# DanielLin94144/E2E-ASR-Pytorch

Hardware: NVIDIA B200
Metric: beam-8+LM joint CTC/attn decode utts/sec (higher is better)
Workload: dtype f32

## Files before the change

### e2e-asr-pytorch_b200/_lib.py

```python
import ctypes
import os

from . import build as _build

c_int, c_float, c_void_p = ctypes.c_int, ctypes.c_float, ctypes.c_void_p

CTC_LOGZERO = -100000000.0
DEC_LOG_ZERO = -10000000.0
STATUS_PREFIX_TOO_LONG = 1
STATUS_TOKEN_NOT_CAND = 2
PREFIX_FULL = 1
PREFIX_SKIP_DEAD_ROWS = 2
PREFIX_FAST_MATH = 4
PREFIX_LIBM_MATH = 8
PREFIX_ROW_COPIES = 16
PREFIX_POLY_MATH = 32
PREFIX_POLY_ESTRIN = 64
BEAM_USE_CTC = 1
BEAM_USE_LM = 2

SIGNATURES = {
    "e2e_last_error": (ctypes.c_char_p, []),
    "e2e_abi_version": (c_int, []),
    "e2e_padded_vocab": (c_int, [c_int]),
# ... 37 lines not shown
    "e2e_lstm_cell": (c_int, [c_void_p, ctypes.c_longlong, c_void_p, c_void_p, c_void_p, c_void_p, c_void_p, c_int, c_int,
                              c_void_p, c_void_p, c_void_p, ctypes.c_longlong, c_int, c_int, c_void_p]),
    "e2e_lstm_split_rows_f16x2": (c_int, [c_void_p, ctypes.c_longlong, c_void_p, c_int, c_int, c_void_p, ctypes.c_longlong, c_int, c_int,
                                          c_float, c_void_p]),
    "e2e_lstm_split_rows_multi_f16x2": (c_int, [c_int, c_void_p, c_void_p, c_void_p, c_void_p, c_void_p, c_void_p, c_void_p, c_void_p,
                                                c_int, c_float, c_void_p]),
    "e2e_lstm_cell_f16x2": (c_int, [c_void_p, ctypes.c_longlong, c_float, c_void_p, c_void_p, c_void_p, c_void_p, c_void_p, c_int, c_int,
                                    c_void_p, c_void_p, c_void_p, ctypes.c_longlong, c_int, c_int, c_float, c_void_p]),
    "e2e_gru_cell": (c_int, [c_void_p, ctypes.c_longlong, c_void_p, c_void_p, c_void_p, c_void_p, c_void_p, c_int, c_int,
                             c_void_p, c_void_p, ctypes.c_longlong, c_int, c_int, c_void_p]),
    "e2e_gru_cell_f16x2": (c_int, [c_void_p, ctypes.c_longlong, c_float, c_void_p, c_void_p, c_void_p, c_void_p, c_void_p, c_int, c_int,
                                   c_void_p, c_void_p, ctypes.c_longlong, c_int, c_int, c_float, c_void_p]),
    "e2e_conv3x3_unfold_split": (c_int, [c_void_p, c_void_p, c_int, c_int, c_int, c_int, ctypes.c_longlong, c_int, c_void_p, c_void_p]),
    "e2e_conv_bias_relu_mask": (c_int, [c_void_p, c_void_p, c_void_p, c_int, c_int, c_int, c_int, ctypes.c_longlong,
                                        ctypes.c_longlong, c_void_p]),
    "e2e_lstm_sequence": (c_int, [c_void_p, ctypes.c_longlong, c_void_p, ctypes.c_longlong, c_void_p, c_void_p, c_void_p, c_void_p,
                                  c_int, c_int, c_int, c_int,
                                  c_void_p, c_void_p, c_int, c_int, c_void_p, c_void_p, c_int, c_int, c_void_p]),
    "e2e_gru_sequence": (c_int, [c_void_p, ctypes.c_longlong, c_void_p, ctypes.c_longlong, c_void_p, c_void_p, c_void_p, c_void_p,
                                 c_int, c_int, c_int, c_int,
                                 c_void_p, c_void_p, c_int, c_int, c_void_p, c_void_p, c_int, c_int, c_void_p]),
    "e2e_conv1_direct": (c_int, [c_void_p, ctypes.c_longlong, c_void_p, c_void_p, c_void_p, c_int, c_int, c_int, c_int, c_int,
                                 c_void_p, c_void_p]),
    "e2e_conv_bias_relu_mask_pool": (c_int, [c_void_p, c_void_p, c_void_p, c_int, c_int, c_int, c_int, c_void_p, c_void_p]),
    "e2e_conv1_direct_amax": (c_int, [c_void_p, ctypes.c_longlong, c_void_p, c_void_p, c_void_p, c_int, c_int, c_int, c_int, c_int,
                                      c_void_p, c_void_p, c_void_p]),
    "e2e_conv3x3_unfold_split_f16x2": (c_int, [c_void_p, c_void_p, c_int, c_int, c_int, c_int, ctypes.c_longlong, c_int, c_void_p,
                                               c_void_p, c_void_p]),
    "e2e_conv_bias_relu_mask_scaled": (c_int, [c_void_p, c_void_p, c_void_p, c_int, c_int, c_int, c_int, ctypes.c_longlong,
                                               ctypes.c_longlong, c_void_p, c_float, c_void_p, c_void_p]),
# ... 53 lines not shown
```

### e2e-asr-pytorch_b200/build.py

```python
import os
import shutil
import subprocess

_HERE = os.path.dirname(os.path.abspath(__file__))
CSRC = os.path.join(_HERE, "csrc")
LIB_DIR = os.path.join(_HERE, "lib")
LIB_PATH = os.path.join(LIB_DIR, "libe2e_asr_b200.so")
SOURCES = ["abi.cu", "ctc_posterior.cu", "prefix_score.cu", "prefix_lazy.cu", "beam_step.cu", "attention_full.cu", "lstm_step.cu", "conv_split.cu", "lstm_seq.cu"]
HEADERS = [os.path.join(CSRC, "common.cuh"), os.path.join(CSRC, "softplus_lut.inc"), os.path.join(CSRC, "softplus_poly.inc"), os.path.join(_HERE, "..", "include", "e2e_asr_b200.h")]
NVCC_FLAGS = ["-gencode", "arch=compute_100a,code=sm_100a", "-O3", "-lineinfo", "-std=c++17",
              "--expt-extended-lambda", "-Xcompiler", "-fPIC", "-shared"]


def _nvcc():
    for cand in (os.environ.get("NVCC"), shutil.which("nvcc"), "/usr/local/cuda/bin/nvcc"):
        if cand and os.path.exists(cand):
            return cand
    return None


def stale():
    if not os.path.exists(LIB_PATH):
        return True
    built = os.path.getmtime(LIB_PATH)
    deps = [os.path.join(CSRC, s) for s in SOURCES] + HEADERS
    return any(os.path.getmtime(d) > built for d in deps)


def build(force=False, verbose=False):
    if not force and not stale():
        return LIB_PATH
    nvcc = _nvcc()
    if nvcc is None:
        raise RuntimeError("nvcc not found: cannot build libe2e_asr_b200.so")
    import tempfile
    from concurrent.futures import ThreadPoolExecutor
    os.makedirs(LIB_DIR, exist_ok=True)
    compile_flags = [f for f in NVCC_FLAGS if f != "-shared"] + (["-Xptxas", "-v"] if verbose else [])
    with tempfile.TemporaryDirectory(prefix="e2e_build_") as tmp:
        def compile_one(src):
            obj = os.path.join(tmp, src.replace(".cu", ".o"))
            proc = subprocess.run([nvcc] + compile_flags + ["-c", "-o", obj, src], cwd=CSRC, capture_output=True, text=True)
            return src, obj, proc
        with ThreadPoolExecutor(max_workers=min(len(SOURCES), os.cpu_count() or 1)) as pool:
            done = list(pool.map(compile_one, SOURCES))
        failed = [(src, proc) for src, _, proc in done if proc.returncode != 0]
        if failed:
            raise RuntimeError("nvcc failed:\n" + "\n".join(src + ":\n" + proc.stdout + proc.stderr for src, proc in failed))
        if verbose:
            for src, _, proc in done:
                print(proc.stderr)
        out_tmp = LIB_PATH + ".tmp%d" % os.getpid()
        link = subprocess.run([nvcc] + NVCC_FLAGS + ["-o", out_tmp] + [obj for _, obj, _ in done], cwd=CSRC, capture_output=True, text=True)
        if link.returncode != 0:
            raise RuntimeError("nvcc link failed:\n" + link.stdout + link.stderr)
        os.replace(out_tmp, LIB_PATH)
    return LIB_PATH


if __name__ == "__main__":
    print(build(force=True, verbose=True))
```

### e2e-asr-pytorch_b200/csrc/prefix_score.cu

```cuda
#include "common.cuh"
#include <stdlib.h>
#include <string.h>
#include <cuda.h>

namespace e2e {

#ifndef E2E_PS_MINBLOCKS
#define E2E_PS_MINBLOCKS 6
#endif
#ifndef E2E_PS_UNROLL
#define E2E_PS_UNROLL 4
#endif
constexpr int kTileBig = 16, kTileSmall = 32;
__host__ __device__ constexpr int phi_pitch(int tile) { return 2 * tile + 2; }
constexpr int kMaxRowFloats = 256;
constexpr int kMaxLanes = 128;
constexpr int kLutBytes = kLutNodes * kLutCopies * 16;
__host__ __device__ constexpr int lut_bytes(int math) { return (math == kMathPoly || math == kMathPolyEstrin) ? 0 : kLutBytes; }

struct PrefixParams {
    const float *x; int Tmax, U, Vp, V;
    const int *enc_len;
    const float2 *r_prev; int lanes_prev;
    const int *prev_lane, *last_tok, *prefix_len, *n_live, *cand;
// ... 238 lines not shown
    }
}

static size_t prefix_smem_bytes(bool gather, int lanes, int Vp, int H, int tile, int math)
{
    size_t b = lut_bytes(math) + prefix_xs_bytes(gather, lanes, Vp, tile) + prefix_phis_bytes(H, tile) + prefix_stage_bytes(H, tile);
    b = ((b + (size_t)(H + 2) * 4 + 7) & ~(size_t)7) + 16;
    return (b + 15) & ~(size_t)15;
}

typedef void (*PrefixKernel)(PrefixParams, CUtensorMap);

typedef CUresult (*EncodeTiledFn)(CUtensorMap *, CUtensorMapDataType, cuuint32_t, void *, const cuuint64_t *, const cuuint64_t *,
                                  const cuuint32_t *, const cuuint32_t *, CUtensorMapInterleave, CUtensorMapSwizzle,
                                  CUtensorMapL2promotion, CUtensorMapFloatOOBfill);
static EncodeTiledFn tensor_map_encoder()
{
    static EncodeTiledFn fn = nullptr;
    static bool tried = false;
    if (!tried) {
        tried = true;
        void *ptr = nullptr;
        cudaDriverEntryPointQueryResult q;
        if (cudaGetDriverEntryPoint("cuTensorMapEncodeTiled", &ptr, cudaEnableDefault, &q) == cudaSuccess && q == cudaDriverEntryPointSuccess)
            fn = reinterpret_cast<EncodeTiledFn>(ptr);
        else
            cudaGetLastError();
    }
    return fn;
}

// ... 117 lines not shown
```

### e2e-asr-pytorch_b200/decode.py

```python
import os

import numpy as np
import torch
import torch.nn.functional as F
import yaml
from torch import nn

from . import _lib as L
from . import ops
from .model import RNNLM
from .stepper import BatchedStepper

CTC_BEAM_RATIO = 1.5
LOG_ZERO = -10000000.0
EOS_THRESHOLD = 1.5


class Hypothesis:

    def __init__(self, tokens, scores, avg):
        self._tokens = np.asarray(tokens, dtype=np.int64)
        self._scores = np.asarray(scores, dtype=np.float32)
        self._avg = np.float32(avg)

# ... 61 lines not shown
            self.lm = RNNLM(self.asr.vocab_size, **cfg['model'])
            self.lm.load_state_dict(torch.load(self.lm_path, map_location='cpu')['model'])
            self.lm.eval()

        self.apply_emb = emb_decoder is not None
        if self.apply_emb:
            raise NotImplementedError("embedding-fusion decoding (src/plugin.py) is outside the decode hot-path scope")

        self.fast_math = False
        self.prefix_math = os.environ.get("E2E_PREFIX_MATH", "poly")
        self.skip_dead_rows = True
        self.lazy_prefix = os.environ.get("E2E_PREFIX_LAZY", "1") != "0"
        self.split_gemm = True
        self.lm_split = os.environ.get("E2E_LM_SPLIT", "bf16x3")
        self.vgg_split = os.environ.get("E2E_VGG_SPLIT", "bf16x3")
        self.fused_attention = True
        self.step_graphs = os.environ.get("E2E_STEP_GRAPHS", "1") != "0"
        self._stepper = None
        self.profile_prefix = False
        self.prefix_events = []
        self.profile_phases = False
        self.phase_ms = {}
        self.last_stats = {}
        self.last_h2d_bytes = 0

    def __getstate__(self):
        d = self.__dict__.copy()
        d["_stepper"], d["prefix_events"] = None, []
        d.pop("_copier", None)
        return d
# ... 115 lines not shown
        n_steps = int(max_len.max()) if n_utts else 0
        n_run = [int((max_np > s).sum()) for s in range(n_steps)]

        marks = []

        coarse = self.profile_phases == "coarse"

        def mark(name, boundary=False):
            if self.profile_phases and (boundary or not coarse):
                e = torch.cuda.Event(enable_timing=True)
                e.record()
                marks.append((name, e))

        with _Fp32Math():
            mark("start", True)
            knobs = (self.split_gemm, self.fused_attention, self.lm_split, self.vgg_split, self.step_graphs)
            if self._stepper is None or self._stepper[0] != dev or self._stepper[1] != knobs:
                self._stepper = (dev, knobs, BatchedStepper(self.asr, self.lm if self.apply_lm else None,
                                                            self.split_gemm, self.fused_attention, self.lm_split, self.vgg_split,
                                                            self.step_graphs))
            stepper = self._stepper[2]
            stepper.mark = mark
            enc, enc_len = stepper.encode(audio_feature, feature_len.to(dev))
            mark("encode", True)
            enc_len32 = enc_len.to(torch.int32).contiguous()
            stepper.start(enc, enc_len, beam)
            t_max = enc.shape[1]
            buf = ops.BeamBuffers(n_utts, beam, n_cand, n_steps, min_len, max_len, dev)
            r_prev = r_a = r_b = x = None
            if self.apply_ctc:
                lin = self.asr.ctc_layer[0]
                logits = F.linear(enc, lin.weight, lin.bias).contiguous()
                x = ops.ctc_log_softmax(logits, enc_len32, apply_relu=True)
                del logits
                r_prev = r_init = ops.ctc_init_state(x, enc_len32)
# ... 97 lines not shown
```

### e2e-asr-pytorch_b200/model.py

```python
import math

import numpy as np
import torch
from torch import nn
import torch.nn.functional as F

FBANK_SIZE = 40


def reference_init_(module):
    if isinstance(module, nn.Embedding):
        module.weight.data.normal_(0, 1)
        return
    for p in module.parameters():
        d = p.data
        if d.dim() == 1:
            d.zero_()
        elif d.dim() == 2:
            d.normal_(0, 1.0 / math.sqrt(d.size(1)))
        elif d.dim() in (3, 4):
            fan = d.size(1)
            for k in d.size()[2:]:
                fan *= k
            d.normal_(0, 1.0 / math.sqrt(fan))
# ... 60 lines not shown
            m = torch.arange(a.shape[2], device=a.device)[None, :] < valid[:, None]
            return a * m[:, None, :, None].to(a.dtype)

        img = keep(img)
        for layer in self.extractor:
            img = layer(img)
            if isinstance(layer, nn.ReLU):
                img = keep(img)
        out = img.transpose(1, 2).contiguous()
        return out.view(out.shape[0], out.shape[1], self.out_dim), feat_len // 4


    A_BYTES = 3 << 30

    conv_split_format = "bf16x3"

    def _split_weights(self, conv):
        from .stepper import SplitLinear, SplitLinearF16
        cache = self.__dict__.setdefault("_split_cache", {})
        key = (id(conv), conv.weight.device, self.conv_split_format)
        if key not in cache:
            w2d = conv.weight.detach().permute(2, 3, 1, 0).reshape(-1, conv.out_channels).t().contiguous()
            cache[key] = SplitLinearF16(w2d, act_scale=1.0) if self.conv_split_format == "fp16x2" else SplitLinear(w2d)
        return cache[key]

    def _conv_split(self, x, valid, conv, pool=False, amax_in=None, amax_out=None):
        from . import ops
        n, h, w, c = x.shape
        k = 9 * c
        lin = self._split_weights(conv)
        total = n * h * w
        f16 = amax_in is not None
        pieces, a_dtype = (2, torch.float16) if f16 else (3, torch.bfloat16)
        blk = max(1, min(total, self.A_BYTES // (pieces * k * 2)))
        a = torch.empty((blk, pieces * k), dtype=a_dtype, device=x.device)
        y = torch.empty((total, conv.out_channels), dtype=torch.float32, device=x.device)
        for p0 in range(0, total, blk):
            m = min(blk, total - p0)
            ops.conv3x3_unfold_split(x, valid, p0, m, a, amax=amax_in)
            am, ym = a[:m], y[p0:p0 + m]
            if f16:
                torch.mm(am, lin.b1, out_dtype=torch.float32, out=ym)
            else:
                torch.mm(am, lin.b2, out_dtype=torch.float32, out=ym)
                torch.addmm(ym, am[:, :2 * k], lin.b1, out_dtype=torch.float32, out=ym)
            torch.addmm(ym, am[:, :k], lin.b0, out_dtype=torch.float32, out=ym)
        y = y.view(n, h, w, conv.out_channels)
        bias = conv.bias.detach().float().contiguous()
        scale_args = (amax_in, lin.out_scale, amax_out) if f16 else ()
        if pool:
            return ops.conv_bias_relu_mask_pool(y, bias, valid, *scale_args)
        ops.conv_bias_relu_mask(y, bias, valid, *scale_args)
        return y

    def forward_masked_split(self, feat, feat_len):
        from . import ops
        drop = feat.shape[1] % 4
        if drop:
            feat = feat[:, :-drop, :]
        if feat.stride(2) != 1 or feat.stride(1) != feat.shape[2]:
            feat = feat.contiguous()
        own = (feat_len // 4 * 4).to(feat.device)
        v1 = own.to(torch.int32).contiguous()
# ... 422 lines not shown
```

### e2e-asr-pytorch_b200/ops.py

```python
import torch

from . import _lib as L

I32, F32 = torch.int32, torch.float32


def _stream():
    return torch.cuda.current_stream().cuda_stream


def _chk(t, dtype, name, numel=None):
    if t is None:
        return
    if not t.is_cuda:
        raise L.E2EError("%s must be a CUDA tensor (no CPU path)" % name)
    if t.dtype != dtype:
        raise TypeError("%s must be %s, got %s" % (name, dtype, t.dtype))
    if not t.is_contiguous():
        raise ValueError("%s must be contiguous" % name)
    if numel is not None and t.numel() < numel:
        raise ValueError("%s has %d elements, needs %d" % (name, t.numel(), numel))


def padded_vocab(v):
# ... 353 lines not shown
def conv3x3_unfold_split(x_nhwc, valid_rows, first_pixel, n_pixels, out, amax=None):
    _chk(x_nhwc, F32, "x_nhwc")
    _chk(valid_rows, I32, "valid_rows", x_nhwc.shape[0])
    n, h, w, c = x_nhwc.shape
    if amax is None:
        _chk(out, torch.bfloat16, "out", n_pixels * 27 * c)
        L.check(L.load().e2e_conv3x3_unfold_split(L.ptr(x_nhwc), L.ptr(valid_rows), n, h, w, c, int(first_pixel), int(n_pixels),
                                                 L.ptr(out), _stream()))
    else:
        _chk(out, torch.float16, "out", n_pixels * 18 * c)
        _chk(amax, I32, "amax", 1)
        L.check(L.load().e2e_conv3x3_unfold_split_f16x2(L.ptr(x_nhwc), L.ptr(valid_rows), n, h, w, c, int(first_pixel), int(n_pixels),
                                                       L.ptr(amax), L.ptr(out), _stream()))


def conv_bias_relu_mask(y_nhwc, bias, valid_rows, amax_in=None, inv_w_scale=None, amax_out=None):
    _chk(y_nhwc, F32, "y_nhwc")
    _chk(bias, F32, "bias", y_nhwc.shape[3])
    _chk(valid_rows, I32, "valid_rows", y_nhwc.shape[0])
    n, h, w, c = y_nhwc.shape
    if amax_in is None:
        L.check(L.load().e2e_conv_bias_relu_mask(L.ptr(y_nhwc), L.ptr(bias), L.ptr(valid_rows), n, h, w, c, 0, n * h * w, _stream()))
    else:
        _chk(amax_in, I32, "amax_in", 1)
        _chk(amax_out, I32, "amax_out", 1)
        L.check(L.load().e2e_conv_bias_relu_mask_scaled(L.ptr(y_nhwc), L.ptr(bias), L.ptr(valid_rows), n, h, w, c, 0, n * h * w,
                                                       L.ptr(amax_in), float(inv_w_scale), L.ptr(amax_out), _stream()))


def lstm_sequence(gates, out, frame_off, lens, group_first, group_rows, hidden, fw, bw=None):
# ... 79 lines not shown
```

### e2e-asr-pytorch_b200/stepper.py

```python
import numpy as np
import torch
import torch.nn.functional as F


def _split3(x):
    a1 = x.to(torch.bfloat16)
    r = x - a1.float()
    a2 = r.to(torch.bfloat16)
    a3 = (r - a2.float()).to(torch.bfloat16)
    return a1, a2, a3


class SplitLinear:

    MIN_ROWS = 1024

    def __init__(self, weight, bias=None):
        self.weight = weight.detach().float()
        self.bias = None if bias is None else bias.detach().float()
        w1, w2, w3 = _split3(self.weight)
        self.b0 = w1.t().contiguous()
        self.b1 = torch.cat([w2, w1], dim=1).t().contiguous()
        self.b2 = torch.cat([w3, w2, w1], dim=1).t().contiguous()

# ... 246 lines not shown
            tail = dict(table=self.table0 if l == 0 else None, tok=tok if (l == 0 and self.table0 is not None) else None,
                        a_next=self.a[l + 1] if nxt else None, k_next=(self.k_in[l + 1] + d) if nxt else 0, off_next=0,
                        gate_scale=lin.out_scale if self.f16 else None, next_scale=self.scale)
            if self.gru:
                ops.gru_cell(y, self.bias[l], self.h[cur][l], idx, n, self.h[new][l], **tail)
            else:
                ops.lstm_cell(y, self.bias[l], self.c[cur][l], idx, n, self.c[new][l], self.h[new][l], **tail)
        self.cur = new
        return self.h[new][self.layers - 1][:n]

    def reorder(self, idx):
        self.idx = idx


class BatchedStepper:
    def __init__(self, asr, lm=None, split_gemm=False, fused_attention=False, lm_split="bf16x3", vgg_split="bf16x3", step_graphs=False):
        att = asr.attention
        if att.mode not in ("loc", "dot"):
            raise NotImplementedError("attention mode " + str(att.mode))
        self.asr, self.lm = asr, lm
        self.split_conv = bool(split_gemm)
        if vgg_split not in ("bf16x3", "fp16x2"):
            raise ValueError("unknown split format " + str(vgg_split))
        self.vgg_split = vgg_split
        self.mode, self.temperature = att.mode, att.att_layer.temperature
        self.H = att.num_head
        def make(rnn, table=None, split="bf16x3"):
            on_gpu = next(rnn.parameters()).is_cuda
            if split_gemm and on_gpu and isinstance(rnn, (torch.nn.LSTM, torch.nn.GRU)):
                return _FusedLstm(rnn, table, split)
            return _Rnn(rnn, split_gemm, table)
        self.dec = make(asr.decoder.layers)
        self.lm_rnn = make(lm.rnn, lm.emb.weight.detach(), lm_split) if lm is not None else None
        for stack in (self.dec, self.lm_rnn):
            if isinstance(stack, _FusedLstm):
                stack.use_graphs = bool(step_graphs)
        self.mark = lambda name: None
        self.fused_attention = self.fused_step = False
        if fused_attention and self.mode == "loc":
            lay = att.att_layer
            if lay.loc_proj.weight.shape[1] <= 12 and lay.loc_proj.weight.shape[0] % 4 == 0:
                self.fused_attention = True
                w_conv = lay.loc_conv.weight.detach()
                self._w_conv = w_conv[:, 0, :].contiguous() if self.H == 1 else w_conv.contiguous()
                self._w_proj = lay.loc_proj.weight.detach().contiguous()
                self._w_energy = lay.gen_energy.weight.detach().reshape(-1).contiguous()
                self._b_energy = float(lay.gen_energy.bias.detach().reshape(-1)[0])

    def encode(self, feats, lens, chunk=128):
        enc_mod = self.asr.encoder
        n_utts = feats.shape[0]
        for layer in getattr(enc_mod, "layers", []):
            if hasattr(layer, "conv_split_format"):
                layer.conv_split_format = self.vgg_split
        packed = (n_utts > 1 and self.split_conv and feats.is_cuda and hasattr(enc_mod, "forward_ragged_packed")
                  and enc_mod.packed_supported())
        ready = getattr(enc_mod, "chunk_ready", None)
        if ready is not None and not packed:
            ready(0, n_utts)
        if n_utts == 1:
            enc, enc_len = enc_mod(feats[:, :int(lens[0])], lens)
        elif packed:
            enc_mod.split_conv = True
            enc, enc_len = enc_mod.forward_ragged_packed(feats, lens, chunk)
        elif hasattr(enc_mod, "forward_ragged"):
            enc_mod.split_conv = self.split_conv and feats.is_cuda
            lens_host = lens.cpu()
            outs, ls = [], []
            for lo in range(0, n_utts, chunk):
# ... 180 lines not shown
```

### include/e2e_asr_b200.h

```cpp
#ifndef E2E_ASR_B200_H
#define E2E_ASR_B200_H

#ifdef __cplusplus
extern "C" {
#endif

#define E2E_ABI_VERSION 1

#define E2E_CTC_LOGZERO   (-100000000.0f)
#define E2E_CTC_BLANK     0
#define E2E_CTC_EOS       1
#define E2E_DEC_LOG_ZERO  (-10000000.0f)

#define E2E_OK              0
#define E2E_ERR_ARG        (-1)
#define E2E_ERR_LAUNCH     (-2)
#define E2E_ERR_UNSUPPORTED (-3)

#define E2E_STATUS_PREFIX_TOO_LONG   1
#define E2E_STATUS_TOKEN_NOT_CAND    2

#define E2E_PREFIX_FULL           1
#define E2E_PREFIX_SKIP_DEAD_ROWS 2
#define E2E_PREFIX_FAST_MATH      4
// ... 91 lines not shown
                        float next_scale, void *stream);

int e2e_gru_cell(const float *gates, long long gates_pitch, const float *bias, const float *table, const long long *tok,
                 const float *h_prev, const long long *row_idx, int n, int D,
                 float *h_new, void *a_next_bf16, long long a_pitch, int K_next, int off_next, void *stream);
int e2e_gru_cell_f16x2(const float *gates, long long gates_pitch, float gate_scale, const float *bias, const float *table,
                       const long long *tok, const float *h_prev, const long long *row_idx, int n, int D,
                       float *h_new, void *a_next_f16, long long a_pitch, int K_next, int off_next, float next_scale, void *stream);

int e2e_conv3x3_unfold_split(const float *in_nhwc, const int *valid_rows, int N, int H, int W, int C,
                             long long first_pixel, int n_pixels, void *out_bf16, void *stream);

int e2e_conv_bias_relu_mask(float *y_nhwc, const float *bias, const int *valid_rows, int N, int H, int W, int C,
                            long long first_pixel, long long n_pixels, void *stream);

int e2e_lstm_sequence(const float *gates, long long gates_pitch, float *out, long long out_pitch,
                      const int *frame_off, const int *lens, const int *group_first, const int *group_rows,
                      int N, int H, int n_groups, int n_dirs,
                      const float *bias_fw, const float *w_t_fw, int gate_off_fw, int out_off_fw,
                      const float *bias_bw, const float *w_t_bw, int gate_off_bw, int out_off_bw,
                      void *stream);

int e2e_gru_sequence(const float *gates, long long gates_pitch, float *out, long long out_pitch,
                     const int *frame_off, const int *lens, const int *group_first, const int *group_rows,
                     int N, int H, int n_groups, int n_dirs,
                     const float *bias_fw, const float *w_t_fw, int gate_off_fw, int out_off_fw,
                     const float *bias_bw, const float *w_t_bw, int gate_off_bw, int out_off_bw,
                     void *stream);

int e2e_conv1_direct(const float *feat, long long feat_pitch_n, const float *weight, const float *bias,
// ... 28 lines not shown
```

Baseline: 1001.

## Add tcgen05 implicit-GEMM 3x3 conv with fused bf16x3 split and epilogue

```diff
diff --git a/e2e-asr-pytorch_b200/_lib.py b/e2e-asr-pytorch_b200/_lib.py
--- a/e2e-asr-pytorch_b200/_lib.py
+++ b/e2e-asr-pytorch_b200/_lib.py
@@ -75,6 +75,8 @@
     "e2e_conv3x3_unfold_split": (c_int, [c_void_p, c_void_p, c_int, c_int, c_int, c_int, ctypes.c_longlong, c_int, c_void_p, c_void_p]),
     "e2e_conv_bias_relu_mask": (c_int, [c_void_p, c_void_p, c_void_p, c_int, c_int, c_int, c_int, ctypes.c_longlong,
                                         ctypes.c_longlong, c_void_p]),
+    "e2e_conv3x3_igemm_supported": (c_int, [c_int, c_int]),
+    "e2e_conv3x3_igemm": (c_int, [c_void_p, c_void_p, c_int, c_int, c_int, c_int, c_void_p, c_void_p, c_int, c_int, c_void_p, c_void_p]),
     "e2e_lstm_sequence": (c_int, [c_void_p, ctypes.c_longlong, c_void_p, ctypes.c_longlong, c_void_p, c_void_p, c_void_p, c_void_p,
                                   c_int, c_int, c_int, c_int,
                                   c_void_p, c_void_p, c_int, c_int, c_void_p, c_void_p, c_int, c_int, c_void_p]),
diff --git a/e2e-asr-pytorch_b200/build.py b/e2e-asr-pytorch_b200/build.py
--- a/e2e-asr-pytorch_b200/build.py
+++ b/e2e-asr-pytorch_b200/build.py
@@ -6,8 +6,11 @@
 CSRC = os.path.join(_HERE, "csrc")
 LIB_DIR = os.path.join(_HERE, "lib")
 LIB_PATH = os.path.join(LIB_DIR, "libe2e_asr_b200.so")
-SOURCES = ["abi.cu", "ctc_posterior.cu", "prefix_score.cu", "prefix_lazy.cu", "beam_step.cu", "attention_full.cu", "lstm_step.cu", "conv_split.cu", "lstm_seq.cu"]
-HEADERS = [os.path.join(CSRC, "common.cuh"), os.path.join(CSRC, "softplus_lut.inc"), os.path.join(CSRC, "softplus_poly.inc"), os.path.join(_HERE, "..", "include", "e2e_asr_b200.h")]
+TC_LIB_PATH = os.path.join(LIB_DIR, "libe2e_asr_b200_tc.so")
+SOURCES = ["abi.cu", "ctc_posterior.cu", "prefix_score.cu", "prefix_lazy.cu", "beam_step.cu", "attention_full.cu", "lstm_step.cu", "conv_split.cu",
+           "conv_igemm_host.cu", "lstm_seq.cu"]
+TC_SOURCES = ["conv_igemm.cu"]
+HEADERS = [os.path.join(CSRC, "common.cuh"), os.path.join(CSRC, "conv_igemm.cuh"), os.path.join(CSRC, "softplus_lut.inc"), os.path.join(CSRC, "softplus_poly.inc"), os.path.join(_HERE, "..", "include", "e2e_asr_b200.h")]
 NVCC_FLAGS = ["-gencode", "arch=compute_100a,code=sm_100a", "-O3", "-lineinfo", "-std=c++17",
               "--expt-extended-lambda", "-Xcompiler", "-fPIC", "-shared"]
 
@@ -20,10 +23,10 @@
 
 
 def stale():
-    if not os.path.exists(LIB_PATH):
+    if not os.path.exists(LIB_PATH) or not os.path.exists(TC_LIB_PATH):
         return True
-    built = os.path.getmtime(LIB_PATH)
-    deps = [os.path.join(CSRC, s) for s in SOURCES] + HEADERS
+    built = min(os.path.getmtime(LIB_PATH), os.path.getmtime(TC_LIB_PATH))
+    deps = [os.path.join(CSRC, s) for s in SOURCES + TC_SOURCES] + HEADERS
     return any(os.path.getmtime(d) > built for d in deps)
 
 
@@ -42,19 +45,25 @@
             obj = os.path.join(tmp, src.replace(".cu", ".o"))
             proc = subprocess.run([nvcc] + compile_flags + ["-c", "-o", obj, src], cwd=CSRC, capture_output=True, text=True)
             return src, obj, proc
-        with ThreadPoolExecutor(max_workers=min(len(SOURCES), os.cpu_count() or 1)) as pool:
-            done = list(pool.map(compile_one, SOURCES))
+        with ThreadPoolExecutor(max_workers=min(len(SOURCES) + len(TC_SOURCES), os.cpu_count() or 1)) as pool:
+            done = list(pool.map(compile_one, SOURCES + TC_SOURCES))
         failed = [(src, proc) for src, _, proc in done if proc.returncode != 0]
         if failed:
             raise RuntimeError("nvcc failed:\n" + "\n".join(src + ":\n" + proc.stdout + proc.stderr for src, proc in failed))
         if verbose:
             for src, _, proc in done:
                 print(proc.stderr)
-        out_tmp = LIB_PATH + ".tmp%d" % os.getpid()
-        link = subprocess.run([nvcc] + NVCC_FLAGS + ["-o", out_tmp] + [obj for _, obj, _ in done], cwd=CSRC, capture_output=True, text=True)
-        if link.returncode != 0:
-            raise RuntimeError("nvcc link failed:\n" + link.stdout + link.stderr)
-        os.replace(out_tmp, LIB_PATH)
+        objs = {src: obj for src, obj, _ in done}
+
+        def link(path, srcs, extra):
+            out_tmp = path + ".tmp%d" % os.getpid()
+            proc = subprocess.run([nvcc] + NVCC_FLAGS + ["-o", out_tmp] + [objs[s] for s in srcs] + extra, cwd=CSRC,
+                                  capture_output=True, text=True)
+            if proc.returncode != 0:
+                raise RuntimeError("nvcc link failed:\n" + proc.stdout + proc.stderr)
+            os.replace(out_tmp, path)
+        link(TC_LIB_PATH, TC_SOURCES, [])
+        link(LIB_PATH, SOURCES, ["-L" + LIB_DIR, "-le2e_asr_b200_tc", "-Xlinker", "-rpath=$ORIGIN"])
     return LIB_PATH
 
 
diff --git a/e2e-asr-pytorch_b200/csrc/conv_igemm.cu b/e2e-asr-pytorch_b200/csrc/conv_igemm.cu
--- /dev/null
+++ b/e2e-asr-pytorch_b200/csrc/conv_igemm.cu
@@ -0,0 +1,305 @@
+#include "common.cuh"
+#include "conv_igemm.cuh"
+#include <cuda_bf16.h>
+
+namespace e2e {
+namespace {
+
+constexpr int kBM = kIgemmBM, kBN = kIgemmBN, kBK = kIgemmBK;
+constexpr int kTile = kBM * kBK * 2;
+constexpr int kBStages = 6;
+constexpr int kBarBytes = 256;
+constexpr int kGroups = 3;
+constexpr int kAStages = 2 * kGroups;
+constexpr int kThreads = 64 + 128 * kGroups;
+constexpr int kSmemBytes = 1024 + (kAStages + kBStages) * kTile + kBarBytes + kBM * 16;
+
+static_assert((2 * (kAStages + kBStages) + 1) * 8 + 4 <= kBarBytes, "barrier block");
+
+constexpr uint32_t kIdesc = (1u << 4) | (1u << 7) | (1u << 10) | ((uint32_t)(kBN >> 3) << 17) | ((uint32_t)(kBM >> 4) << 24);
+
+__device__ __forceinline__ uint64_t sw128_desc(uint32_t saddr)
+{
+    return (uint64_t)((saddr >> 4) & 0x3fffu) | ((uint64_t)1 << 16) | ((uint64_t)(1024 >> 4) << 32) | ((uint64_t)1 << 46) |
+           ((uint64_t)2 << 61);
+}
+
+__device__ __forceinline__ void mbar_arrive(uint64_t *bar)
+{
+    asm volatile("mbarrier.arrive.shared::cta.b64 _, [%0];" ::"r"(smem_u32(bar)) : "memory");
+}
+
+__device__ __forceinline__ void tma_load_2d(void *dst, const CUtensorMap *map, int c0, int c1, uint64_t *bar)
+{
+    asm volatile("cp.async.bulk.tensor.2d.shared::cluster.global.tile.mbarrier::complete_tx::bytes [%0], [%1, {%2, %3}], [%4];"
+                 ::"r"(smem_u32(dst)), "l"(map), "r"(c0), "r"(c1), "r"(smem_u32(bar))
+                 : "memory");
+}
+
+__device__ __forceinline__ void tc_fence_after() { asm volatile("tcgen05.fence::after_thread_sync;" ::: "memory"); }
+__device__ __forceinline__ void tc_fence_before() { asm volatile("tcgen05.fence::before_thread_sync;" ::: "memory"); }
+
+__device__ __forceinline__ void tc_mma(uint32_t d_tmem, uint64_t adesc, uint64_t bdesc, uint32_t accumulate)
+{
+    asm volatile("{\n\t.reg .pred p;\n\tsetp.ne.b32 p, %4, 0;\n\t"
+                 "tcgen05.mma.cta_group::1.kind::f16 [%0], %1, %2, %3, p;\n\t}"
+                 ::"r"(d_tmem), "l"(adesc), "l"(bdesc), "r"(kIdesc), "r"(accumulate));
+}
+
+__device__ __forceinline__ void tc_commit(uint64_t *bar)
+{
+    asm volatile("tcgen05.commit.cta_group::1.mbarrier::arrive::one.shared::cluster.b64 [%0];" ::"r"(smem_u32(bar)) : "memory");
+}
+
+__device__ __forceinline__ void tmem_ld32(uint32_t taddr, float (&v)[32])
+{
+    uint32_t *r = reinterpret_cast<uint32_t *>(v);
+    asm volatile("tcgen05.ld.sync.aligned.32x32b.x32.b32 {%0, %1, %2, %3, %4, %5, %6, %7, %8, %9, %10, %11, %12, %13, %14, %15, "
+                 "%16, %17, %18, %19, %20, %21, %22, %23, %24, %25, %26, %27, %28, %29, %30, %31}, [%32];"
+                 : "=r"(r[0]), "=r"(r[1]), "=r"(r[2]), "=r"(r[3]), "=r"(r[4]), "=r"(r[5]), "=r"(r[6]), "=r"(r[7]),
+                   "=r"(r[8]), "=r"(r[9]), "=r"(r[10]), "=r"(r[11]), "=r"(r[12]), "=r"(r[13]), "=r"(r[14]), "=r"(r[15]),
+                   "=r"(r[16]), "=r"(r[17]), "=r"(r[18]), "=r"(r[19]), "=r"(r[20]), "=r"(r[21]), "=r"(r[22]), "=r"(r[23]),
+                   "=r"(r[24]), "=r"(r[25]), "=r"(r[26]), "=r"(r[27]), "=r"(r[28]), "=r"(r[29]), "=r"(r[30]), "=r"(r[31])
+                 : "r"(taddr));
+}
+
+__device__ __forceinline__ uint32_t split_piece2(float x0, float x1, int pp)
+{
+    __nv_bfloat162 p = __floats2bfloat162_rn(x0, x1);
+    if (pp > 0) {
+        const float2 a = __bfloat1622float2(p);
+        x0 = __fsub_rn(x0, a.x);
+        x1 = __fsub_rn(x1, a.y);
+        p = __floats2bfloat162_rn(x0, x1);
+        if (pp > 1) {
+            const float2 b = __bfloat1622float2(p);
+            p = __floats2bfloat162_rn(__fsub_rn(x0, b.x), __fsub_rn(x1, b.y));
+        }
+    }
+    return *reinterpret_cast<uint32_t *>(&p);
+}
+
+struct alignas(16) IgemmRow {
+    const float *pix;
+    uint32_t flags;
+    uint32_t pad;
+};
+constexpr uint32_t kRowLive = 1u << 9, kRowPixel = 1u << 10;
+
+__global__ void __launch_bounds__(kThreads, 1)
+conv3x3_igemm_kernel(const __grid_constant__ CUtensorMap wmap, const IgemmArgs args)
+{
+    extern __shared__ uint8_t igemm_smem_raw[];
+    uint8_t *smem = reinterpret_cast<uint8_t *>((reinterpret_cast<uintptr_t>(igemm_smem_raw) + 1023) & ~(uintptr_t)1023);
+    uint8_t *a_ring = smem;
+    uint8_t *b_ring = smem + kAStages * kTile;
+    uint64_t *bars = reinterpret_cast<uint64_t *>(b_ring + kBStages * kTile);
+    uint64_t *a_full = bars, *a_empty = bars + kAStages;
+    uint64_t *b_full = bars + 2 * kAStages, *b_empty = b_full + kBStages;
+    uint64_t *acc_full = b_empty + kBStages;
+    uint32_t *tmem_slot = reinterpret_cast<uint32_t *>(acc_full + 1);
+    IgemmRow *rows = reinterpret_cast<IgemmRow *>(reinterpret_cast<uint8_t *>(bars) + kBarBytes);
+
+    const int warp = threadIdx.x >> 5, lane = threadIdx.x & 31;
+    const int H = args.H, W = args.W, C = args.C;
+    const bool pool = args.epi == kEpiPool;
+    const int n0 = blockIdx.y * kBN;
+    const int KB = 9 * C / kBK;
+
+    if (threadIdx.x == 0) {
+        for (int i = 0; i < kAStages; ++i) { mbar_init(a_full + i, 128); mbar_init(a_empty + i, 1); }
+        for (int i = 0; i < kBStages; ++i) { mbar_init(b_full + i, 1); mbar_init(b_empty + i, 1); }
+        mbar_init(acc_full, 1);
+        mbar_fence_init();
+    }
+    if (warp == 0) {
+        asm volatile("tcgen05.alloc.cta_group::1.sync.aligned.shared::cta.b32 [%0], 512;" ::"r"(smem_u32(tmem_slot)) : "memory");
+        asm volatile("tcgen05.relinquish_alloc_permit.cta_group::1.sync.aligned;" ::: "memory");
+    }
+    if (threadIdx.x >= 64 && threadIdx.x < 64 + kBM) {
+        const int m = threadIdx.x - 64;
+        int h = 0, w = 0, n = -1;
+        if (pool) {
+            const int H2 = (H + 1) >> 1, W2 = (W + 1) >> 1;
+            const long long q = (long long)blockIdx.x * (kBM / 4) + (m >> 2);
+            if (q < (long long)args.N * H2 * W2) {
+                const int w2 = (int)(q % W2);
+                const long long t = q / W2;
+                h = 2 * (int)(t % H2) + ((m >> 1) & 1);
+                w = 2 * w2 + (m & 1);
+                if (h < H && w < W) n = (int)(t / H2);
+            }
+        } else {
+            const long long p = (long long)blockIdx.x * kBM + m;
+            if (p < (long long)args.N * H * W) {
+                const long long t = p / W;
+                w = (int)(p % W);
+                h = (int)(t % H);
+                n = (int)(t / H);
+            }
+        }
+        IgemmRow r = {args.in, 0u, 0u};
+        if (n >= 0) {
+            const int vr = __ldg(args.valid + n);
+            r.pix = args.in + (((long long)n * H + h) * W + w) * C;
+            r.flags = kRowPixel | (h < vr ? kRowLive : 0u);
+            for (int t = 0; t < 9; ++t) {
+                const int hs = h + t / 3 - 1, ws = w + t % 3 - 1;
+                if (hs >= 0 && hs < H && hs < vr && ws >= 0 && ws < W) r.flags |= 1u << t;
+            }
+        }
+        rows[m] = r;
+    }
+    tc_fence_before();
+    __syncthreads();
+    tc_fence_after();
+    const uint32_t tmem = *tmem_slot;
+
+    if (warp == 0) {
+        if (lane == 0) {
+            int stage = 0;
+            uint32_t phase = 0;
+            for (int pp = 0; pp < 3; ++pp)
+                for (int kb = 0; kb < KB; ++kb)
+                    for (int j = 0; j < 3 - pp; ++j) {
+                        mbar_wait(b_empty + stage, phase ^ 1u);
+                        mbar_arrive_expect_tx(b_full + stage, kTile);
+                        tma_load_2d(b_ring + stage * kTile, &wmap, kb * kBK, j * args.Cout + n0, b_full + stage);
+                        if (++stage == kBStages) { stage = 0; phase ^= 1u; }
+                    }
+        }
+    } else if (warp == 1) {
+        if (lane == 0) {
+            int as = 0, bs = 0;
+            uint32_t aph = 0, bph = 0;
+            for (int pp = 0; pp < 3; ++pp)
+                for (int kb = 0; kb < KB; ++kb) {
+                    mbar_wait(a_full + as, aph);
+                    tc_fence_after();
+                    const uint64_t adesc = sw128_desc(smem_u32(a_ring + as * kTile));
+                    for (int j = 0; j < 3 - pp; ++j) {
+                        mbar_wait(b_full + bs, bph);
+                        tc_fence_after();
+                        const uint64_t bdesc = sw128_desc(smem_u32(b_ring + bs * kTile));
+#pragma unroll
+                        for (int k16 = 0; k16 < kBK / 16; ++k16)
+                            tc_mma(tmem + (uint32_t)((pp + j) * kBN), adesc + 2 * k16, bdesc + 2 * k16,
+                                   (pp > 0 || kb > 0 || k16 > 0) ? 1u : 0u);
+                        tc_commit(b_empty + bs);
+                        if (++bs == kBStages) { bs = 0; bph ^= 1u; }
+                    }
+                    tc_commit(a_empty + as);
+                    if (++as == kAStages) { as = 0; aph ^= 1u; }
+                }
+            tc_commit(acc_full);
+        }
+    } else {
+        const int grp = (threadIdx.x - 64) >> 7, pt = (threadIdx.x - 64) & 127;
+        const int c16 = pt & 15, rsub = pt >> 4;
+        const int cpb = C / kBK;
+        int as = grp;
+        uint32_t aph = 0;
+        for (int seq = grp; seq < 3 * KB; seq += kGroups) {
+            const int pp = seq / KB, kb = seq - pp * KB, tap = kb / cpb, cb = kb - tap * cpb;
+            const long long tap_off = ((long long)(tap / 3 - 1) * W + (tap % 3 - 1)) * C + cb * kBK + c16 * 4;
+            float4 v[kBM / 8];
+#pragma unroll
+            for (int i = 0; i < kBM / 8; ++i) {
+                const IgemmRow r = rows[i * 8 + rsub];
+                v[i] = make_float4(0.0f, 0.0f, 0.0f, 0.0f);
+                if ((r.flags >> tap) & 1u) v[i] = __ldg(reinterpret_cast<const float4 *>(r.pix + tap_off));
+            }
+            mbar_wait(a_empty + as, aph ^ 1u);
+            uint8_t *tile = a_ring + as * kTile;
+#pragma unroll
+            for (int i = 0; i < kBM / 8; ++i) {
+                const int row = i * 8 + rsub;
+                const uint32_t lo = split_piece2(v[i].x, v[i].y, pp), hi = split_piece2(v[i].z, v[i].w, pp);
+                const int chunk = (c16 >> 1) ^ (row & 7);
+                *reinterpret_cast<uint2 *>(tile + row * 128 + chunk * 16 + (c16 & 1) * 8) = make_uint2(lo, hi);
+            }
+            asm volatile("fence.proxy.async.shared::cta;" ::: "memory");
+            mbar_arrive(a_full + as);
+            as += kGroups;
+            if (as >= kAStages) { as -= kAStages; aph ^= 1u; }
+        }
+
+        const int m = (warp & 3) * 32 + lane;
+        const uint32_t flags = rows[m].flags;
+        mbar_wait(acc_full, 0);
+        tc_fence_after();
+        const uint32_t lane_addr = tmem + ((uint32_t)((warp & 3) * 32) << 16);
+        const long long H2W2 = (long long)((H + 1) >> 1) * ((W + 1) >> 1);
+        const bool live = (flags & kRowLive) != 0u, pixel = (flags & kRowPixel) != 0u;
+        for (int c = grp; c < kBN / 32; c += kGroups) {
+            float y0[32], y1[32], y2[32];
+            tmem_ld32(lane_addr + c * 32, y0);
+            tmem_ld32(lane_addr + kBN + c * 32, y1);
+            tmem_ld32(lane_addr + 2 * kBN + c * 32, y2);
+            asm volatile("tcgen05.wait::ld.sync.aligned;" ::: "memory");
+            float y[32];
+#pragma unroll
+            for (int i = 0; i < 32; ++i) y[i] = __fadd_rn(y0[i], __fadd_rn(y1[i], y2[i]));
+            const int col = n0 + c * 32;
+            if (args.epi == kEpiRaw) {
+                if (pixel) {
+                    float4 *dst = reinterpret_cast<float4 *>(args.out + ((long long)blockIdx.x * kBM + m) * args.Cout + col);
+#pragma unroll
+                    for (int i = 0; i < 8; ++i) dst[i] = make_float4(y[4 * i], y[4 * i + 1], y[4 * i + 2], y[4 * i + 3]);
+                }
+            } else if (!pool) {
+                if (pixel) {
+                    float4 *dst = reinterpret_cast<float4 *>(args.out + ((long long)blockIdx.x * kBM + m) * args.Cout + col);
+#pragma unroll
+                    for (int i = 0; i < 8; ++i) {
+                        float4 o = make_float4(0.0f, 0.0f, 0.0f, 0.0f);
+                        if (live) {
+                            const float4 b = __ldg(reinterpret_cast<const float4 *>(args.bias + col) + i);
+                            o.x = fmaxf(__fadd_rn(y[4 * i], b.x), 0.0f); o.y = fmaxf(__fadd_rn(y[4 * i + 1], b.y), 0.0f);
+                            o.z = fmaxf(__fadd_rn(y[4 * i + 2], b.z), 0.0f); o.w = fmaxf(__fadd_rn(y[4 * i + 3], b.w), 0.0f);
+                        }
+                        dst[i] = o;
+                    }
+                }
+            } else {
+                const int s = m & 3, base = lane & ~3;
+                float t[32];
+#pragma unroll
+                for (int i = 0; i < 32; ++i) t[i] = live ? __fadd_rn(y[i], __ldg(args.bias + col + i)) : -INFINITY;
+                float res[8];
+#pragma unroll
+                for (int i = 0; i < 32; ++i) {
+                    float acc = 0.0f;
+#pragma unroll
+                    for (int k = 0; k < 4; ++k) acc = fmaxf(acc, __shfl_sync(E2E_FULL_MASK, t[i], base + k));
+                    if ((i >> 3) == s) res[i & 7] = acc;
+                }
+                const long long q = (long long)blockIdx.x * (kBM / 4) + (m >> 2);
+                if (q < (long long)args.N * H2W2) {
+                    float4 *dst = reinterpret_cast<float4 *>(args.out + q * args.Cout + col + 8 * s);
+                    dst[0] = make_float4(res[0], res[1], res[2], res[3]);
+                    dst[1] = make_float4(res[4], res[5], res[6], res[7]);
+                }
+            }
+        }
+        tc_fence_before();
+    }
+    __syncthreads();
+    if (warp == 0) asm volatile("tcgen05.dealloc.cta_group::1.sync.aligned.b32 %0, 512;" ::"r"(tmem) : "memory");
+}
+
+}
+}
+
+extern "C" int e2e_tc_conv3x3_igemm_launch(const CUtensorMap *wmap, const e2e::IgemmArgs *args, unsigned tiles, void *stream)
+{
+    using namespace e2e;
+    static bool attr_set = false;
+    if (!attr_set) {
+        const cudaError_t e = cudaFuncSetAttribute(conv3x3_igemm_kernel, cudaFuncAttributeMaxDynamicSharedMemorySize, kSmemBytes);
+        if (e != cudaSuccess) return (int)e;
+        attr_set = true;
+    }
+    conv3x3_igemm_kernel<<<dim3(tiles, (unsigned)(args->Cout / kBN)), kThreads, kSmemBytes, static_cast<cudaStream_t>(stream)>>>(*wmap, *args);
+    return (int)cudaGetLastError();
+}
diff --git a/e2e-asr-pytorch_b200/csrc/conv_igemm.cuh b/e2e-asr-pytorch_b200/csrc/conv_igemm.cuh
--- /dev/null
+++ b/e2e-asr-pytorch_b200/csrc/conv_igemm.cuh
@@ -0,0 +1,23 @@
+#pragma once
+#include <cuda.h>
+#include <cuda_runtime.h>
+
+namespace e2e {
+
+constexpr int kIgemmBM = 128;
+constexpr int kIgemmBN = 128;
+constexpr int kIgemmBK = 64;
+
+enum { kEpiRaw = 0, kEpiRelu = 1, kEpiPool = 2 };
+
+struct IgemmArgs {
+    const float *in;
+    const int *valid;
+    const float *bias;
+    float *out;
+    int N, H, W, C, Cout, epi;
+};
+
+}
+
+extern "C" int e2e_tc_conv3x3_igemm_launch(const CUtensorMap *wmap, const e2e::IgemmArgs *args, unsigned tiles, void *stream);
diff --git a/e2e-asr-pytorch_b200/csrc/conv_igemm_host.cu b/e2e-asr-pytorch_b200/csrc/conv_igemm_host.cu
--- /dev/null
+++ b/e2e-asr-pytorch_b200/csrc/conv_igemm_host.cu
@@ -0,0 +1,61 @@
+#include "common.cuh"
+#include "conv_igemm.cuh"
+
+namespace e2e {
+
+typedef CUresult (*EncodeTiledFn)(CUtensorMap *, CUtensorMapDataType, cuuint32_t, void *, const cuuint64_t *, const cuuint64_t *,
+                                  const cuuint32_t *, const cuuint32_t *, CUtensorMapInterleave, CUtensorMapSwizzle,
+                                  CUtensorMapL2promotion, CUtensorMapFloatOOBfill);
+EncodeTiledFn tensor_map_encoder();
+
+namespace {
+
+bool igemm_shape_ok(int C, int Cout)
+{
+    return (C == 128 || C == 256) && (Cout == 128 || Cout == 256);
+}
+
+}
+}
+
+using namespace e2e;
+
+extern "C" int e2e_conv3x3_igemm_supported(int C, int Cout)
+{
+    return igemm_shape_ok(C, Cout) ? 1 : 0;
+}
+
+extern "C" int e2e_conv3x3_igemm(const float *in_nhwc, const int *valid_rows, int N, int H, int W, int C,
+                                 const void *w_split_bf16, const float *bias, int Cout, int epilogue, float *out, void *stream)
+{
+    const char *name = "e2e_conv3x3_igemm";
+    if (!in_nhwc || !valid_rows || !w_split_bf16 || !out || (epilogue != kEpiRaw && !bias))
+        return set_error(E2E_ERR_ARG, "%s: null pointer", name);
+    if (N <= 0 || H <= 0 || W <= 0 || epilogue < kEpiRaw || epilogue > kEpiPool)
+        return set_error(E2E_ERR_ARG, "%s: bad size or epilogue", name);
+    if (!igemm_shape_ok(C, Cout)) return set_error(E2E_ERR_UNSUPPORTED, "%s: C = %d, Cout = %d not supported", name, C, Cout);
+    if ((reinterpret_cast<uintptr_t>(in_nhwc) & 15) || (reinterpret_cast<uintptr_t>(w_split_bf16) & 15) ||
+        (reinterpret_cast<uintptr_t>(out) & 15) || (reinterpret_cast<uintptr_t>(bias) & 15))
+        return set_error(E2E_ERR_ARG, "%s: misaligned buffer", name);
+    const long long rows_out = epilogue == kEpiPool ? (long long)N * ((H + 1) / 2) * ((W + 1) / 2) : (long long)N * H * W;
+    const long long tiles = epilogue == kEpiPool ? (rows_out + kIgemmBM / 4 - 1) / (kIgemmBM / 4) : (rows_out + kIgemmBM - 1) / kIgemmBM;
+    if (tiles > 0x7fffffffLL) return set_error(E2E_ERR_ARG, "%s: too many pixels", name);
+
+    EncodeTiledFn enc = tensor_map_encoder();
+    if (!enc) return set_error(E2E_ERR_LAUNCH, "%s: cuTensorMapEncodeTiled is not available from this driver", name);
+    CUtensorMap map;
+    const cuuint64_t dims[2] = {(cuuint64_t)9 * C, (cuuint64_t)3 * Cout};
+    const cuuint64_t strides[1] = {(cuuint64_t)9 * C * 2};
+    const cuuint32_t box[2] = {(cuuint32_t)kIgemmBK, (cuuint32_t)kIgemmBN};
+    const cuuint32_t estr[2] = {1u, 1u};
+    const CUresult cr = enc(&map, CU_TENSOR_MAP_DATA_TYPE_BFLOAT16, 2, const_cast<void *>(w_split_bf16), dims, strides, box, estr,
+                            CU_TENSOR_MAP_INTERLEAVE_NONE, CU_TENSOR_MAP_SWIZZLE_128B, CU_TENSOR_MAP_L2_PROMOTION_L2_256B,
+                            CU_TENSOR_MAP_FLOAT_OOB_FILL_NONE);
+    if (cr != CUDA_SUCCESS) return set_error(E2E_ERR_LAUNCH, "%s: cuTensorMapEncodeTiled failed (CUresult %d)", name, (int)cr);
+
+    const IgemmArgs a = {in_nhwc, valid_rows, bias, out, N, H, W, C, Cout, epilogue};
+    const int e = e2e_tc_conv3x3_igemm_launch(&map, &a, (unsigned)tiles, stream);
+    count_launch();
+    if (e != (int)cudaSuccess) return set_error(E2E_ERR_LAUNCH, "%s: %s", name, cudaGetErrorString((cudaError_t)e));
+    return check_launch(name);
+}
diff --git a/e2e-asr-pytorch_b200/csrc/prefix_score.cu b/e2e-asr-pytorch_b200/csrc/prefix_score.cu
--- a/e2e-asr-pytorch_b200/csrc/prefix_score.cu
+++ b/e2e-asr-pytorch_b200/csrc/prefix_score.cu
@@ -276,7 +276,7 @@
 typedef CUresult (*EncodeTiledFn)(CUtensorMap *, CUtensorMapDataType, cuuint32_t, void *, const cuuint64_t *, const cuuint64_t *,
                                   const cuuint32_t *, const cuuint32_t *, CUtensorMapInterleave, CUtensorMapSwizzle,
                                   CUtensorMapL2promotion, CUtensorMapFloatOOBfill);
-static EncodeTiledFn tensor_map_encoder()
+EncodeTiledFn tensor_map_encoder()
 {
     static EncodeTiledFn fn = nullptr;
     static bool tried = false;
diff --git a/e2e-asr-pytorch_b200/decode.py b/e2e-asr-pytorch_b200/decode.py
--- a/e2e-asr-pytorch_b200/decode.py
+++ b/e2e-asr-pytorch_b200/decode.py
@@ -99,6 +99,7 @@
         self.split_gemm = True
         self.lm_split = os.environ.get("E2E_LM_SPLIT", "bf16x3")
         self.vgg_split = os.environ.get("E2E_VGG_SPLIT", "bf16x3")
+        self.vgg_conv = "igemm"
         self.fused_attention = True
         self.step_graphs = os.environ.get("E2E_STEP_GRAPHS", "1") != "0"
         self._stepper = None
@@ -244,11 +245,11 @@
 
         with _Fp32Math():
             mark("start", True)
-            knobs = (self.split_gemm, self.fused_attention, self.lm_split, self.vgg_split, self.step_graphs)
+            knobs = (self.split_gemm, self.fused_attention, self.lm_split, self.vgg_split, self.step_graphs, self.vgg_conv)
             if self._stepper is None or self._stepper[0] != dev or self._stepper[1] != knobs:
                 self._stepper = (dev, knobs, BatchedStepper(self.asr, self.lm if self.apply_lm else None,
                                                             self.split_gemm, self.fused_attention, self.lm_split, self.vgg_split,
-                                                            self.step_graphs))
+                                                            self.step_graphs, self.vgg_conv))
             stepper = self._stepper[2]
             stepper.mark = mark
             enc, enc_len = stepper.encode(audio_feature, feature_len.to(dev))
diff --git a/e2e-asr-pytorch_b200/model.py b/e2e-asr-pytorch_b200/model.py
--- a/e2e-asr-pytorch_b200/model.py
+++ b/e2e-asr-pytorch_b200/model.py
@@ -98,6 +98,8 @@
     A_BYTES = 3 << 30
 
     conv_split_format = "bf16x3"
+    conv_path = "igemm"
+    IGEMM_MAX_COUT = 128
 
     def _split_weights(self, conv):
         from .stepper import SplitLinear, SplitLinearF16
@@ -108,9 +110,21 @@
             cache[key] = SplitLinearF16(w2d, act_scale=1.0) if self.conv_split_format == "fp16x2" else SplitLinear(w2d)
         return cache[key]
 
+    def _igemm_weights(self, conv):
+        cache = self.__dict__.setdefault("_split_cache", {})
+        key = (id(conv), conv.weight.device, "igemm")
+        if key not in cache:
+            lin, k = self._split_weights(conv), 9 * conv.in_channels
+            cache[key] = torch.stack([lin.b0.t(), lin.b1[:k].t(), lin.b2[:k].t()]).contiguous()
+        return cache[key]
+
     def _conv_split(self, x, valid, conv, pool=False, amax_in=None, amax_out=None):
         from . import ops
         n, h, w, c = x.shape
+        bias = conv.bias.detach().float().contiguous()
+        if (amax_in is None and self.conv_path == "igemm" and conv.out_channels <= self.IGEMM_MAX_COUT
+                and ops.conv3x3_igemm_supported(c, conv.out_channels)):
+            return ops.conv3x3_igemm(x, valid, self._igemm_weights(conv), bias, "pool" if pool else "relu")
         k = 9 * c
         lin = self._split_weights(conv)
         total = n * h * w
@@ -130,7 +144,6 @@
                 torch.addmm(ym, am[:, :2 * k], lin.b1, out_dtype=torch.float32, out=ym)
             torch.addmm(ym, am[:, :k], lin.b0, out_dtype=torch.float32, out=ym)
         y = y.view(n, h, w, conv.out_channels)
-        bias = conv.bias.detach().float().contiguous()
         scale_args = (amax_in, lin.out_scale, amax_out) if f16 else ()
         if pool:
             return ops.conv_bias_relu_mask_pool(y, bias, valid, *scale_args)
diff --git a/e2e-asr-pytorch_b200/ops.py b/e2e-asr-pytorch_b200/ops.py
--- a/e2e-asr-pytorch_b200/ops.py
+++ b/e2e-asr-pytorch_b200/ops.py
@@ -391,6 +391,37 @@
                                                        L.ptr(amax), L.ptr(out), _stream()))
 
 
+def conv3x3_igemm_supported(c_in, c_out):
+    return bool(L.load().e2e_conv3x3_igemm_supported(int(c_in), int(c_out)))
+
+
+IGEMM_EPILOGUE = {"raw": 0, "relu": 1, "pool": 2}
+
+
+def conv3x3_igemm(x_nhwc, valid_rows, w_split, bias, epilogue="relu"):
+    _chk(x_nhwc, F32, "x_nhwc")
+    _chk(valid_rows, I32, "valid_rows", x_nhwc.shape[0])
+    _chk(w_split, torch.bfloat16, "w_split")
+    n, h, w, c = x_nhwc.shape
+    if w_split.dim() != 3 or w_split.shape[0] != 3 or w_split.shape[2] != 9 * c:
+        raise ValueError("w_split must be [3, Cout, 9*%d], got %s" % (c, tuple(w_split.shape)))
+    cout = w_split.shape[1]
+    if epilogue not in IGEMM_EPILOGUE:
+        raise ValueError("unknown epilogue " + str(epilogue))
+    if epilogue != "raw":
+        _chk(bias, F32, "bias", cout)
+    if epilogue == "raw":
+        out = torch.empty((n * h * w, cout), dtype=F32, device=x_nhwc.device)
+    elif epilogue == "relu":
+        out = torch.empty((n, h, w, cout), dtype=F32, device=x_nhwc.device)
+    else:
+        out = torch.empty((n, (h + 1) // 2, (w + 1) // 2, cout), dtype=F32, device=x_nhwc.device)
+    L.check(L.load().e2e_conv3x3_igemm(L.ptr(x_nhwc), L.ptr(valid_rows), n, h, w, c, L.ptr(w_split),
+                                      L.ptr(bias) if epilogue != "raw" else None, int(cout), IGEMM_EPILOGUE[epilogue],
+                                      L.ptr(out), _stream()))
+    return out
+
+
 def conv_bias_relu_mask(y_nhwc, bias, valid_rows, amax_in=None, inv_w_scale=None, amax_out=None):
     _chk(y_nhwc, F32, "y_nhwc")
     _chk(bias, F32, "bias", y_nhwc.shape[3])
diff --git a/e2e-asr-pytorch_b200/stepper.py b/e2e-asr-pytorch_b200/stepper.py
--- a/e2e-asr-pytorch_b200/stepper.py
+++ b/e2e-asr-pytorch_b200/stepper.py
@@ -284,7 +284,8 @@
 
 
 class BatchedStepper:
-    def __init__(self, asr, lm=None, split_gemm=False, fused_attention=False, lm_split="bf16x3", vgg_split="bf16x3", step_graphs=False):
+    def __init__(self, asr, lm=None, split_gemm=False, fused_attention=False, lm_split="bf16x3", vgg_split="bf16x3", step_graphs=False,
+                 vgg_conv="igemm"):
         att = asr.attention
         if att.mode not in ("loc", "dot"):
             raise NotImplementedError("attention mode " + str(att.mode))
@@ -293,6 +294,9 @@
         if vgg_split not in ("bf16x3", "fp16x2"):
             raise ValueError("unknown split format " + str(vgg_split))
         self.vgg_split = vgg_split
+        if vgg_conv not in ("igemm", "unfold"):
+            raise ValueError("unknown VGG convolution path " + str(vgg_conv))
+        self.vgg_conv = vgg_conv
         self.mode, self.temperature = att.mode, att.att_layer.temperature
         self.H = att.num_head
         def make(rnn, table=None, split="bf16x3"):
@@ -323,6 +327,7 @@
         for layer in getattr(enc_mod, "layers", []):
             if hasattr(layer, "conv_split_format"):
                 layer.conv_split_format = self.vgg_split
+                layer.conv_path = self.vgg_conv
         packed = (n_utts > 1 and self.split_conv and feats.is_cuda and hasattr(enc_mod, "forward_ragged_packed")
                   and enc_mod.packed_supported())
         ready = getattr(enc_mod, "chunk_ready", None)
diff --git a/include/e2e_asr_b200.h b/include/e2e_asr_b200.h
--- a/include/e2e_asr_b200.h
+++ b/include/e2e_asr_b200.h
@@ -129,6 +129,10 @@
 int e2e_conv_bias_relu_mask(float *y_nhwc, const float *bias, const int *valid_rows, int N, int H, int W, int C,
                             long long first_pixel, long long n_pixels, void *stream);
 
+int e2e_conv3x3_igemm_supported(int C, int Cout);
+int e2e_conv3x3_igemm(const float *in_nhwc, const int *valid_rows, int N, int H, int W, int C,
+                      const void *w_split_bf16, const float *bias, int Cout, int epilogue, float *out, void *stream);
+
 int e2e_lstm_sequence(const float *gates, long long gates_pitch, float *out, long long out_pitch,
                       const int *frame_off, const int *lens, const int *group_first, const int *group_rows,
                       int N, int H, int n_groups, int n_dirs,
```

Measured after the change: 1034, median of 6. +3.3%, better.
